# ArrowLuo/SegCLIP

Measured on AMD Instinct MI355X. Metric: image-text pairs/s fwd+bwd, ViT-B/16 224^2, per-GPU batch 256 (global 2048 at 8 GPUs), higher is better.
Workload: dtype bf16; 1 GPU; BASELINE configs[1]/[2]: ViT-B/16 224^2 + 77-token text, contrastive loss only; per_gpu_batch=256, global_batch=256, parallelism=dp1, attention_forward=bf16, residual_stream=fp32, cross_mode=t18, text_positions=all 77 (full context, as the reference computes it)

## Files before the change

### include/segclip_hip.h

```cpp
#ifndef SEGCLIP_HIP_H
#define SEGCLIP_HIP_H

#include <stddef.h>
#include <stdint.h>

#ifdef __cplusplus
extern "C" {
#endif

#define SEGCLIP_ABI_VERSION 1

#define SEGCLIP_F32 0
#define SEGCLIP_BF16 1

#define SEGCLIP_ACT_NONE 0
#define SEGCLIP_ACT_QUICK_GELU 1
#define SEGCLIP_ACT_GELU_ERF 2

#define SEGCLIP_ERR_INVALID (-1)
#define SEGCLIP_ERR_UNSUPPORTED (-2)

int segclip_version(void);
const char* segclip_last_error_string(void);

// ... 68 lines not shown
int segclip_layernorm_fwd_multi(const void* x, int n, const float* const* gamma, const float* const* beta,
                                void* const* y, const int64_t* maps, float* mean, float* rstd, int64_t rows,
                                int64_t cols, float eps, int x_dtype, int y_dtype, void* stream);
size_t segclip_layernorm_bwd_multi_ws_bytes(int64_t rows, int64_t cols, int n);
int segclip_layernorm_bwd_multi(const void* const* dy, const void* x, int n, const float* const* gamma,
                                const int64_t* maps, const float* mean, const float* rstd, void* dx, float* dgb,
                                void* ws, int64_t rows, int64_t cols, int dy_dtype, int x_dtype, void* stream);

#define SEGCLIP_ATTN_FP8 1
typedef struct segclip_attn_desc {
  const void* Q;
  const void* K;
  const void* V;
  void* O;
  void* stats;
  const void* dO;
  void* dQ;
  void* dK;
  void* dV;
  void* ws;
  int64_t B, H, Tq, Tk, hd;
  int64_t q_sb, q_st, k_sb, k_st, v_sb, v_st, o_sb, o_st;
  int64_t dq_sb, dq_st, dk_sb, dk_st, dv_sb, dv_st, do_sb, do_st;
  float scale;
  int32_t causal;
  int32_t dtype;
  int32_t flags;
  void* colsum_part;
  const int32_t* klen;
} segclip_attn_desc;

size_t segclip_attn_stats_bytes(const segclip_attn_desc* d);
size_t segclip_attn_bwd_ws_bytes(const segclip_attn_desc* d);
int segclip_attn_fwd(const segclip_attn_desc* d, void* stream);
int segclip_attn_bwd(const segclip_attn_desc* d, void* stream);

typedef struct segclip_resblock_fwd_desc {
  const void* x;
  const float* ln1w; const float* ln1b; const void* wqkv; const float* bqkv; const void* wo; const float* bo;
  const float* ln2w; const float* ln2b; const void* wfc; const float* bfc; const void* wpr; const float* bpr;
  void* y1; float* mean1; float* rstd1;
  void* qkv;
  void* o;
  void* stats;
  void* x1;
  void* y2; float* mean2; float* rstd2;
  void* h; int64_t ld_h;
  void* u; int64_t ld_u;
  void* xo;
  const void* klen;
  int64_t M, B, T, D, F, H;
  float eps, attn_scale;
  int32_t causal, act, aux_kind, x_dtype;
} segclip_resblock_fwd_desc;
int segclip_resblock_fwd(const segclip_resblock_fwd_desc* d, void* stream);

int segclip_cast(const void* src, void* dst, int64_t n, int src_dtype, int dst_dtype, void* stream);
int segclip_split3_bf16(const float* src, void* dst, int64_t rows, int64_t cols, int64_t ld, int stack, int role, void* stream);
size_t segclip_colsum_ws_bytes(int64_t M, int64_t N);
int segclip_colsum(const void* X, float* out, void* ws, int64_t M, int64_t N, int64_t ld, int dtype,
                   void* stream);
int segclip_act_fwd(const void* x, void* y, int64_t n, int act, int dtype, void* stream);
int segclip_act_bwd(const void* dy, const void* x, void* dx, int64_t n, int act, int dtype, void* stream);
int segclip_add(const void* a, const void* b, void* out, int64_t n, int dtype, void* stream);

int segclip_im2col(const float* image, void* cols, int64_t B, int64_t C, int64_t H, int64_t W, int64_t p,
                   int layout, int out_dtype, void* stream);
int segclip_im2col_ld(const float* image, void* cols, int64_t B, int64_t C, int64_t H, int64_t W, int64_t p,
                      int layout, int out_dtype, int64_t ld, void* stream);
int segclip_vis_assemble(const void* patches, const float* cls, const float* pos, float* x, int64_t B,
                         int64_t T, int64_t D, int p_dtype, void* stream);

int segclip_embed_fwd(const int64_t* ids, const float* table, const float* pos, float* out, int64_t B,
                      int64_t L, int64_t D, int64_t vocab, void* stream);
int segclip_embed_bwd(const int64_t* ids, const float* dout, float* dtable, float* dpos, int64_t B,
                      int64_t L, int64_t D, int64_t vocab, void* stream);

int segclip_mean_cat_fwd(const float* x, float* out, int64_t B, int64_t T, int64_t D, void* stream);
int segclip_mean_cat_bwd(const float* dout, float* dx, int64_t B, int64_t T, int64_t D, void* stream);
int segclip_mae_unshuffle_fwd(const float* x, const float* mask_token, const int64_t* ids, const float* pos, float* out, int64_t B,
                              int64_t K, int64_t L, int64_t D, void* stream);
int segclip_mae_unshuffle_bwd(const float* dout, const int64_t* ids, float* dx, float* dpos, float* mpart, int64_t B, int64_t K,
                              int64_t L, int64_t D, void* stream);

int segclip_gather_rows(const void* src, const int64_t* idx, void* out, int64_t B, int64_t Tsrc,
                        int64_t Tout, int64_t D, int dtype, void* stream);
int segclip_scatter_rows(const void* dout, const int64_t* idx, void* dsrc, int64_t B, int64_t Tsrc,
                         int64_t Tout, int64_t D, int dtype, void* stream);

int segclip_assign_fwd(const float* logits, const float* gumbel, float tau, float* y_soft, float* soft,
                       uint8_t* idx, float* hard, float* counts, int64_t B, int64_t G, int64_t T,
                       void* stream);
int segclip_assign_bwd(const float* dhard, const float* y_soft, float tau, float* dlogits, int64_t B,
                       int64_t G, int64_t T, void* stream);

int segclip_l2norm_fwd(const float* x, float* y, float* norm, int64_t rows, int64_t cols, void* stream);
int segclip_l2norm_bwd(const float* dy, const float* y, const float* norm, float* dx, int64_t rows,
                       int64_t cols, void* stream);
int segclip_ce_fwd(const float* logits, float* lse, float* loss_rows, int64_t rows, int64_t cols,
                   int64_t label_offset, void* stream);
int segclip_ce_bwd(const float* logits, const float* lse, const float* gscale_ptr, float gscale,
                   float* dlogits, int64_t rows, int64_t cols, int64_t label_offset, void* stream);
int segclip_ce_labels_fwd(const float* logits, const int64_t* labels, int64_t ignore_index, float* lse, float* loss_rows,
                          float* valid, int64_t rows, int64_t cols, void* stream);
int segclip_ce_labels_bwd(const float* logits, const float* lse, const int64_t* labels, int64_t ignore_index,
                          const float* gscale, const float* inv_count, float* dlogits, int64_t rows, int64_t cols,
                          void* stream);
int segclip_superpixel_kl(const float* hard, const int64_t* seg, float* loss_rows, float* dhard,
// ... 330 lines not shown
```

### segclip_amd/config.py

```python
import contextlib
import sys
import threading
import types

import torch

_warned_env = set()


def tuning_env(name, default):
    import os
    v = os.environ.get(name)
    if v is None:
        return default
    if os.environ.get("SEGCLIP_TUNING", "0") in ("", "0"):
        if name not in _warned_env:
            _warned_env.add(name)
            print(f"segclip_amd: {name}={v} ignored (tuning switches need SEGCLIP_TUNING=1)", file=sys.stderr)
        return default
    return v


_DEFAULTS = dict(compute_dtype=torch.float32, f32_split=False, c_exec=tuning_env("SEGCLIP_C_EXEC", "1") != "0", cross_mode="t18", overlap_towers=True,
                 trust_weight_shadows=False, attn_fp8=False, fuse_res_stack=True, bf16_resgrad=True, bf16_resid=False, fused_head=True,
                 aux_u8=tuning_env("SEGCLIP_AUX_U8", "1") != "0",
                 text_after_blocks=3, text_trim=False, text_trim_hint=None, pad_rows=tuning_env("SEGCLIP_PAD_ROWS", "1") != "0", fold_param_grads=tuning_env("SEGCLIP_FOLD_GRADS", "1") != "0",
                 wgrad_group_blocks=int(tuning_env("SEGCLIP_WGRAD_GROUP", "12")), wgrad_group_blocks_dist=int(tuning_env("SEGCLIP_WGRAD_GROUP_DIST", "12")))
_tls = threading.local()


def _get(name):
    ov = getattr(_tls, "overrides", None)
    if ov:
        for d in reversed(ov):
            if name in d:
                return d[name]
    return _DEFAULTS[name]


def _check(name, value):
    if name == "compute_dtype" and value not in (torch.float32, torch.bfloat16):
        raise ValueError("compute dtype must be torch.float32 or torch.bfloat16")
    if name == "cross_mode" and value not in ("t18", "intended"):
        raise ValueError("cross_mode must be 't18' or 'intended'")
    return value


class _ConfigModule(types.ModuleType):
    """Module type whose switches are properties: reads resolve thread-local overrides first, writes set the
    process default."""


for _n in _DEFAULTS:
    setattr(_ConfigModule, _n, property(lambda self, _n=_n: _get(_n),
                                        lambda self, v, _n=_n: _DEFAULTS.__setitem__(_n, _check(_n, v))))
sys.modules[__name__].__class__ = _ConfigModule


def set_compute_dtype(dtype):
    _DEFAULTS["compute_dtype"] = _check("compute_dtype", dtype)


def set_cross_mode(mode):
    _DEFAULTS["cross_mode"] = _check("cross_mode", mode)


@contextlib.contextmanager
def scope(**overrides):
    for k, v in overrides.items():
        if k not in _DEFAULTS:
            raise KeyError(f"unknown switch {k!r}")
        _check(k, v)
    stack = getattr(_tls, "overrides", None)
    if stack is None:
        stack = _tls.overrides = []
    stack.append(dict(overrides))
    try:
        yield
    finally:
        stack.pop()


def set_stack_hook(after_blocks, fn):
    _tls.stack_hook = (int(after_blocks), fn)


def take_stack_hook():
    h = getattr(_tls, "stack_hook", None)
    _tls.stack_hook = None
    return h


@contextlib.contextmanager
def noise_injection(items):
    prev = getattr(_tls, "noise", None)
    _tls.noise = list(items)
    try:
        yield
    finally:
        _tls.noise = prev


def _take(kind, shape, device):
    noise = getattr(_tls, "noise", None)
    if noise is None:
        return None
    if not noise:
        raise RuntimeError("noise_injection: more noise draws than injected tensors")
    k, t = noise.pop(0)
    if k != kind or tuple(t.shape) != tuple(shape):
        raise RuntimeError(f"noise_injection: expected {kind}{tuple(shape)}, got {k}{tuple(t.shape)}")
    return t.to(device=device, dtype=torch.float32)


def gumbel(shape, device):
    t = _take("gumbel", shape, device)
    if t is not None:
        return t
    u = torch.rand(shape, device=device, dtype=torch.float32)
    if u.is_cuda:
        from . import _lib as L
        L.check(L.load().segclip_gumbel_from_uniform(L.ptr(u), L.ptr(u), u.numel(), L.stream()), "gumbel_from_uniform")
        return u
    tiny = torch.finfo(torch.float32).tiny
    u = u.clamp(min=tiny, max=1.0 - torch.finfo(torch.float32).eps)
    return -torch.log(-torch.log(u))


def rand(shape, device):
    t = _take("rand", shape, device)
    if t is not None:
        return t
    return torch.rand(shape, device=device, dtype=torch.float32)
```

### segclip_amd/csrc/exec.cpp

```cpp
#include <initializer_list>

#include "common.h"
#include "gemm_plan.h"

namespace {

void gemm_base(segclip_gemm_desc& g, const void* A, int64_t lda, const void* W, int64_t ldw, void* Cc, int64_t ldc, int c_dtype,
               const float* bias, int64_t M, int64_t N, int64_t K) {
  g = segclip_gemm_desc{};
  g.A = A; g.B = W; g.C = Cc; g.bias = bias;
  g.M = M; g.N = N; g.K = K;
  g.sam = lda; g.sak = 1; g.sbn = ldw; g.sbk = 1;
  g.ldc = ldc; g.ldaux = N;
  g.nb1 = 1; g.nb2 = 1;
  g.a_dtype = SEGCLIP_BF16; g.b_dtype = SEGCLIP_BF16; g.c_dtype = c_dtype; g.r_dtype = SEGCLIP_F32;
  g.act = SEGCLIP_ACT_NONE; g.alpha = 1.0f;
}

}

extern "C" int segclip_resblock_fwd(const segclip_resblock_fwd_desc* d, void* stream) {
  SEGCLIP_REQUIRE(d != nullptr, "resblock_fwd: null descriptor");
  SEGCLIP_REQUIRE(d->M >= d->B * d->T && d->B > 0 && d->T > 0 && d->D > 0 && d->F > 0 && d->H > 0 && d->D % d->H == 0,
                  "resblock_fwd: bad sizes");
  SEGCLIP_REQUIRE(d->x && d->y1 && d->qkv && d->o && d->stats && d->x1 && d->y2 && d->h && d->xo && d->mean1 && d->rstd1 &&
                  d->mean2 && d->rstd2, "resblock_fwd: null buffer");
  SEGCLIP_REQUIRE(d->x_dtype == SEGCLIP_F32 || d->x_dtype == SEGCLIP_BF16, "resblock_fwd: residual stream must be f32 or bf16");
  const int64_t M = d->M, D = d->D, F = d->F, hd = D / d->H;
  segclip_gemm_desc in_proj, out_proj, c_fc, c_proj;
  gemm_base(in_proj, d->y1, D, d->wqkv, D, d->qkv, 3 * D, SEGCLIP_BF16, d->bqkv, M, 3 * D, D);
  gemm_base(out_proj, d->o, D, d->wo, D, d->x1, D, d->x_dtype, d->bo, M, D, D);
  out_proj.residual = d->x; out_proj.ldr = D; out_proj.r_dtype = d->x_dtype;
  gemm_base(c_fc, d->y2, D, d->wfc, D, d->h, d->ld_h, SEGCLIP_BF16, d->bfc, M, F, D);
  c_fc.act = d->act; c_fc.aux = d->u; c_fc.ldaux = d->u ? d->ld_u : F; c_fc.aux_kind = d->aux_kind;
  gemm_base(c_proj, d->h, d->ld_h, d->wpr, F, d->xo, D, d->x_dtype, d->bpr, M, D, F);
  c_proj.residual = d->x1; c_proj.ldr = D; c_proj.r_dtype = d->x_dtype;
  int rc;
  for (const segclip_gemm_desc* g : {&in_proj, &out_proj, &c_fc, &c_proj})
    if ((rc = gemm_plan(g).rc)) return rc;
  rc = segclip_layernorm_fwd(d->x, d->ln1w, d->ln1b, d->y1, d->mean1, d->rstd1, M, D, d->eps, d->x_dtype, SEGCLIP_BF16, stream);
  if (rc) return rc;
  if ((rc = segclip_gemm(&in_proj, stream))) return rc;
  if (M > d->B * d->T) {
    hipError_t e = hipMemsetAsync((char*)d->o + (size_t)d->B * d->T * D * 2, 0, (size_t)(M - d->B * d->T) * D * 2, (hipStream_t)stream);
    SEGCLIP_REQUIRE(e == hipSuccess, "resblock_fwd: memset failed: %s", hipGetErrorString(e));
  }
  segclip_attn_desc a = segclip_attn_desc{};
  a.Q = d->qkv; a.K = (const char*)d->qkv + (size_t)D * 2; a.V = (const char*)d->qkv + (size_t)2 * D * 2; a.O = d->o;
  a.stats = d->stats;
  a.B = d->B; a.H = d->H; a.Tq = d->T; a.Tk = d->T; a.hd = hd;
  a.q_sb = a.k_sb = a.v_sb = d->T * 3 * D; a.q_st = a.k_st = a.v_st = 3 * D;
  a.o_sb = d->T * D; a.o_st = D;
  a.scale = d->attn_scale; a.causal = d->causal; a.dtype = SEGCLIP_BF16; a.flags = 0;
  a.klen = (decltype(a.klen))d->klen;
  if ((rc = segclip_attn_fwd(&a, stream))) return rc;
  if ((rc = segclip_gemm(&out_proj, stream))) return rc;
  rc = segclip_layernorm_fwd(d->x1, d->ln2w, d->ln2b, d->y2, d->mean2, d->rstd2, M, D, d->eps, d->x_dtype, SEGCLIP_BF16, stream);
  if (rc) return rc;
  if ((rc = segclip_gemm(&c_fc, stream))) return rc;
  return segclip_gemm(&c_proj, stream);
}
```

### segclip_amd/modules/modeling.py

```python
from functools import partial

import torch
from torch import nn

from .. import _lib as L
from .. import config, ops
from .module_clip import CLIP, available_models
from .module_mae import MAEDecoder
from .util_module import CrossEn, PreTrainedModel, dist_collect, get_attr, get_logger, show_log


def _detached(obj):
    if isinstance(obj, torch.Tensor):
        return obj.detach()
    if isinstance(obj, dict):
        return {k: _detached(v) for k, v in obj.items()}
    if isinstance(obj, (list, tuple)):
        return type(obj)(_detached(v) for v in obj)
    return obj


class SegCLIPPreTrainedModel(PreTrainedModel, nn.Module):
    def __init__(self, *inputs, **kwargs):
        super().__init__()
# ... 75 lines not shown
        mae_vis_mask_ratio = get_attr(task_config, "mae_vis_mask_ratio", default_value=0.75)
        self.use_vision_mae_recon = get_attr(task_config, "use_vision_mae_recon", default_value=False)
        if self.use_vision_mae_recon:
            self.vis_mask_ratio = mae_vis_mask_ratio
            self.vis_mae_decoder = MAEDecoder(vision_width, vision_width // 2, image_resolution, vision_patch_size,
                                              decoder_depth=3, decoder_num_heads=8, mlp_ratio=4.,
                                              norm_layer=partial(nn.LayerNorm, eps=1e-6))
        mae_seq_mask_ratio = get_attr(task_config, "mae_seq_mask_ratio", default_value=0.15)
        self.use_text_mae_recon = get_attr(task_config, "use_text_mae_recon", default_value=False)
        if self.use_text_mae_recon:
            self.seq_mask_ratio = mae_seq_mask_ratio
            self.seq_mae_decoder = MAEDecoder(embed_dim, embed_dim // 2, image_resolution, vision_patch_size,
                                              decoder_depth=3, decoder_num_heads=8, mlp_ratio=4., choice_seq=True,
                                              pred_len=vocab_size, seq_len=self.task_config.max_words)
        self.use_seglabel = get_attr(task_config, "use_seglabel", default_value=False)
        self.apply(self.init_weights)
        self.segclip_config = {}

    def scope(self):
        return config.scope(**self.segclip_config)

    def _text_stream(self):
        from .. import streams
        return streams.side_stream("text")

    def _visual_feature(self, image, image_frame):
        if config.fused_head:
            return self.clip.encode_image_pooled(image)
        visual_output, _hidden, mid_states = self.get_visual_output(image, shaped=True, image_frame=image_frame, return_hidden=True)
        return visual_output, mid_states

    def forward(self, input_ids, token_type_ids, attention_mask, image, image_seg=None):
        if self.segclip_config:
            with config.scope(**self.segclip_config):
                return self._forward(input_ids, token_type_ids, attention_mask, image, image_seg)
        return self._forward(input_ids, token_type_ids, attention_mask, image, image_seg)

    def _forward(self, input_ids, token_type_ids, attention_mask, image, image_seg=None):
        input_ids = input_ids.view(-1, input_ids.shape[-1])
        L.require_cuda(input_ids, torch.as_tensor(image))
        image_input = torch.as_tensor(image).float()
        b, pair, channel, h, w = image_input.shape
        image = image_input[:, 0].reshape(b, channel, h, w)
        image_frame = 1
        if not self.training:
            return None
        ops._GradFold.advance()
        if config.compute_dtype == torch.bfloat16:
            ops.refresh_weight_shadows(force=not config.trust_weight_shadows)
        if config.overlap_towers:
            main = torch.cuda.current_stream()
            side = self._text_stream()
            ready = torch.cuda.Event()
            ready.record(main)
            box = {}

            def enqueue_text():
                side.wait_event(ready)
                with torch.cuda.stream(side):
                    box["seq"] = self.clip.encode_text_eot(input_ids).unsqueeze(1)
            k = int(config.text_after_blocks)
            if k > 0:
                config.set_stack_hook(k, enqueue_text)
            else:
                enqueue_text()
            pending = None
            try:
                visual_output, mid_states = self._visual_feature(image, image_frame)
                pending = config.take_stack_hook()
            finally:
                config.take_stack_hook()
            if pending is not None:
                pending[1]()
            sequence_output = box["seq"]
            main.wait_stream(side)
            sequence_output.record_stream(main)
        else:
            sequence_output = self.clip.encode_text_eot(input_ids).unsqueeze(1)
            visual_output, mid_states = self._visual_feature(image, image_frame)
        self.last_mid_states = _detached(mid_states)
        self._last_head = {}
        if config.fused_head:
            loss = ops.ClipLossFn.apply(visual_output.float().view(b, -1), sequence_output.squeeze(1).float(),
                                        self.clip.logit_scale, int(getattr(self.task_config, "rank", 0)), self._last_head)
        else:
            sim_matrix_t2v, sim_matrix_v2t = self._loose_similarity(sequence_output, visual_output)
            offset = sequence_output.size(0) * int(getattr(self.task_config, "rank", 0))
            sim_loss1 = ops.CrossEntropyFn.apply(sim_matrix_t2v, offset)
            sim_loss2 = ops.CrossEntropyFn.apply(sim_matrix_v2t, offset)
            loss = (sim_loss1 + sim_loss2) / 2.
            self._last_head["logits"] = (sim_matrix_t2v.detach(), sim_matrix_v2t.detach())
        self.last_losses = {"contrastive": loss.detach()}
        if self.use_seglabel:
            image_seg_ = torch.as_tensor(image_seg)[:, 0].reshape(b, -1)
            hard = mid_states["attns"][0]["hard_attn"]
            clutering_loss = ops.SuperpixelKLFn.apply(hard, image_seg_)
            loss = loss + clutering_loss
            self.last_losses["kl"] = clutering_loss.detach()
        if self.use_text_mae_recon:
            attention_mask = attention_mask.view(-1, attention_mask.shape[-1])
            _, seq_hidden, seq_mae_mask, seq_mae_ids_restore = self.get_sequence_output(
                input_ids, token_type_ids, attention_mask, shaped=True, return_hidden=True, mask_ratio=self.seq_mask_ratio)
            seq_mae_mask = seq_mae_mask.view(-1, seq_mae_mask.size(-1))
            seq_mae_ids_restore = seq_mae_ids_restore.view(-1, seq_mae_ids_restore.size(-1))
            _mae_mask = (seq_mae_mask + attention_mask).gt(1)
            self.last_text_mae = _detached((seq_mae_mask, seq_mae_ids_restore, seq_hidden))
            seq_mae_loss = self.seq_mae_decoder.forward_seq(input_ids, seq_hidden, _mae_mask, seq_mae_ids_restore,
                                                            attention_mask)
            loss = loss + seq_mae_loss
            self.last_losses["text_mae"] = seq_mae_loss.detach()
        if self.use_vision_mae_recon:
            _, vis_hidden, vis_mae_mask, vis_mae_ids_restore, mid_mae_states = self.get_visual_output(
                image, shaped=True, image_frame=image_frame, return_hidden=True, mask_ratio=self.vis_mask_ratio)
            vis_hidden = mid_mae_states["hidden"]
            vis_hidden = ops.mean_cat(vis_hidden)
            vis_mae_mask = vis_mae_mask.view(-1, vis_mae_mask.size(-1))
            vis_mae_ids_restore = vis_mae_ids_restore.view(-1, vis_mae_ids_restore.size(-1))
            self.last_mae = _detached((vis_mae_mask, vis_mae_ids_restore, mid_mae_states))
            vis_mae_loss = self.vis_mae_decoder.forward_vis(image, vis_hidden, vis_mae_mask, vis_mae_ids_restore,
                                                            loss_allpatch=False)
            loss = loss + vis_mae_loss
            self.last_losses["mae"] = vis_mae_loss.detach()
        return loss

    @property
# ... 85 lines not shown
```

### segclip_amd/ops.py

```python
import collections
import ctypes as C
import math
import os
import weakref

import torch
import torch.distributed as dist
from torch.autograd import Function

from . import _lib as L
from . import config as _cfg

ACT_NONE, ACT_QUICK_GELU, ACT_GELU_ERF = L.ACT_NONE, L.ACT_QUICK_GELU, L.ACT_GELU_ERF


class _GemmProfile:
    enabled = False
    records = []

    @classmethod
    def start(cls):
        cls.enabled, cls.records = True, []

    @classmethod
# ... 874 lines not shown
    try:
        L.check(L.load().segclip_resblock_fwd(C.byref(d), L.stream()), "resblock_fwd")
    except L.Unsupported:
        return False
    return True


def _resblock_fwd(x2, P, B, T, n_head, causal, act, eps, act_dtype, klen):
    P = BlockParams._make(P)
    M, D = x2.shape
    F4 = P.wfc.shape[0]
    for w in P:
        sl = _slot_of(w)
        if sl is not None:
            sl.note_forward_use()
    bf = act_dtype == torch.bfloat16
    fp8 = bf and bool(_cfg.attn_fp8)
    wqkv_c, wo_c, wfc_c, wpr_c = (wcast(w, act_dtype) for w in (P.wqkv, P.wo, P.wfc, P.wpr))
    ak = _aux_kind(act_dtype, act, M, F4)
    hidden = _empty_pitched if bf else _empty
    y1, y2, o = (_empty((M, D), act_dtype, x2) for _ in range(3))
    qkv = _empty((M, 3 * D), act_dtype, x2)
    mean1, rstd1, mean2, rstd2 = _empty((4, M), torch.float32, x2).unbind(0)
    x1, xo = _empty((M, D), x2.dtype, x2), _empty((M, D), x2.dtype, x2)
    h = hidden((M, F4), act_dtype, x2)
    u = hidden((M, F4), torch.uint8 if ak == 2 else act_dtype, x2) if act != ACT_NONE else None
    ad = attn_desc_packed(qkv, o, B, n_head, T, causal, klen=klen, fp8=fp8)
    stats = _empty((max(L.load().segclip_attn_stats_bytes(C.byref(ad)) // 4, 1),), torch.float32, x2)
    s = BlockSaved(x=x2, ln1w=P.ln1w, mean1=mean1, rstd1=rstd1, y1=y1, wqkv=wqkv_c, qkv=qkv, o=o, stats=stats, wo=wo_c, x1=x1,
                   ln2w=P.ln2w, mean2=mean2, rstd2=rstd2, y2=y2, wfc=wfc_c, u=u, h=h, wpr=wpr_c)
    if (bf and _cfg.c_exec and not _OpCount.enabled and not _GemmProfile.enabled and not fp8 and x2.is_contiguous() and D % 8 == 0
            and _resblock_fwd_exec(s, P, xo, B, T, n_head, causal, act, eps, klen, ak)):
        return xo, s
    p_ln_fwd(x2, P.ln1w, P.ln1b, eps, act_dtype, out=y1, stats=(mean1, rstd1))
    p_linear(y1, wqkv_c, P.bqkv, out=qkv)
    if M > B * T:
        o[B * T:].zero_()
    p_attn_fwd(ad, x2, stats=stats)
    p_linear(o, wo_c, P.bo, residual=x2, out=x1)
    p_ln_fwd(x1, P.ln2w, P.ln2b, eps, act_dtype, out=y2, stats=(mean2, rstd2))
    _, u = p_linear(y2, wfc_c, P.bfc, act=act, want_aux=True, aux_kind=ak, pitched=bf, out=h, aux_out=u)
    p_linear(h, wpr_c, P.bpr, residual=x1, out=xo)
    return xo, s._replace(u=u)


def _aux_kind(act_dtype, act, M=0, N=0):
    if act_dtype == torch.bfloat16 and act in (ACT_QUICK_GELU, ACT_GELU_ERF):
        if _cfg.aux_u8 and M > 0 and M % 128 == 0 and N % 256 == 0:
            return 2
        return 1 if act == ACT_QUICK_GELU else 0
    return 0


def _resblock_bwd(s, cfg, klen, slots, need, g, g16, chain, wgroup=None, rqueue=None):
    B, T, D, n_head, causal, act, act_dtype = cfg
    M = s.x.shape[0]
    bf = act_dtype == torch.bfloat16
    if bf and g16 is None:
        g16 = p_cast(g, act_dtype)
    if not bf:
        g16 = g
    res_in = g16 if chain else g
    rdt = act_dtype if chain else torch.float32
    F4 = s.wfc.shape[0]

    rq = ReduceQueue() if rqueue is None else rqueue

    def wgrad(dy_, x_, out_):
        if wgroup is not None:
            return wgroup.add(dy_, x_, out_)
        return p_wgrad(dy_, x_, out=out_, defer=rq)

    def vec_out(slot, wanted, n):
        return _slot_out(slot, (n,)) if wanted else None
    du, dbfc = p_dgrad(g16, s.wpr, act_dtype, aux=s.u, act=act, want_colsum=True, colsum_out=vec_out(slots.bfc, need.bfc, F4),
                       aux_kind=2 if s.u.dtype == torch.uint8 else _aux_kind(act_dtype, act),
                       defer=rq, pitched=bf)
    dwpr = wgrad(g16, s.h, _slot_out(slots.wpr, (D, F4))) if need.wpr else None
    dy2 = p_dgrad(du, s.wfc, act_dtype)
    dwfc = wgrad(du, s.y2, _slot_out(slots.wfc, (F4, D))) if need.wfc else None
    two = bf and not chain
    r = p_ln_bwd(dy2, s.x1, s.ln2w, s.mean2, s.rstd2, dres=res_in, dx_dtype=rdt, want_bf16=two, want_dres_colsum=True,
                 outs=(vec_out(slots.ln2w, need.ln2w, D), vec_out(slots.ln2b, need.ln2b, D), vec_out(slots.bpr, need.bpr, D)), defer=rq)
    dx1, dln2w, dln2b = r[0], r[1], r[2]
    dx1_16 = r[3] if two else dx1
    dbpr = r[-1] if need.bpr else None
    do = p_dgrad(dx1_16, s.wo, act_dtype)
    dwo = wgrad(dx1_16, s.o, _slot_out(slots.wo, (D, D))) if need.wo else None
    dqkv = _empty((M, 3 * D), act_dtype, s.x)
    if M > B * T:
        dqkv[B * T:].zero_()
    s3 = (T * 3 * D, 3 * D)
    ad = attn_desc_packed(s.qkv, s.o, B, n_head, T, causal, klen=klen)
    part = _empty((B, 3 * D), torch.float32, s.x) if (bf and need.bqkv) else None
    p_attn_bwd(ad, s.stats, do, dqkv, dqkv, dqkv, s3, s3, s3, (T * D, D), 0, D, 2 * D, colsum_part=part)
    dy1 = p_dgrad(dqkv, s.wqkv, act_dtype)
    dwqkv = wgrad(dqkv, s.y1, _slot_out(slots.wqkv, (3 * D, D))) if need.wqkv else None
    dbqkv = None
    if need.bqkv:
        bq_out = _slot_out(slots.bqkv, (3 * D,))
        if part is not None and (bq_out is None or bq_out.data_ptr() % 16 == 0):
            dbqkv = bq_out if bq_out is not None else _empty((3 * D,), torch.float32, s.x)
            rq.add_rows(part, B, 3 * D, 3 * D, (dbqkv,), 3 * D)
        else:
            dbqkv = p_colsum(part if part is not None else dqkv, out=bq_out)
    r = p_ln_bwd(dy1, s.x, s.ln1w, s.mean1, s.rstd1, dres=dx1, dx_dtype=rdt, want_bf16=two, want_dres_colsum=True,
                 outs=(vec_out(slots.ln1w, need.ln1w, D), vec_out(slots.ln1b, need.ln1b, D), vec_out(slots.bo, need.bo, D)), defer=rq)
    if rqueue is None:
        rq.flush()
    dbo = r[-1] if need.bo else None
    dx32 = None if chain else r[0]
    dx16 = r[0] if chain else (r[3] if two else None)
    return dx32, dx16, BlockParams(ln1w=r[1], ln1b=r[2], wqkv=dwqkv, bqkv=dbqkv, wo=dwo, bo=dbo, ln2w=dln2w, ln2b=dln2b, wfc=dwfc,
                                   bfc=dbfc, wpr=dwpr, bpr=dbpr)


def _bf16_side_copy(g):
    st = getattr(g, "_segclip_bf16", None)
    if st is not None and (st.numel() != g.numel() or st.device != g.device or not g.is_contiguous()):
        return None
    return st


def _pad_rows(t, Mp):
    M = t.shape[0]
    padded = _empty((Mp, t.shape[1]), t.dtype, t)
    padded[:M].copy_(t)
    padded[M:].zero_()
    return padded


class ResBlockFn(Function):

    @staticmethod
    def forward(ctx, x, ln1w, ln1b, wqkv, bqkv, wo, bo, ln2w, ln2b, wfc, bfc, wpr, bpr, n_head, causal, act, eps,
                act_dtype, klen=None):
        B, T, D = x.shape
        x2 = x.contiguous().view(B * T, D)
        P = BlockParams(ln1w, ln1b, wqkv, bqkv, wo, bo, ln2w, ln2b, wfc, bfc, wpr, bpr)
        xo, saved = _resblock_fwd(x2, P, B, T, n_head, causal, act, eps, act_dtype, klen)
        ctx.save_for_backward(*saved)
        ctx.cfg = (B, T, D, n_head, causal, act, act_dtype)
        ctx.klen = klen
        ctx.slots = BlockParams._make(_slot_of(w) for w in P)
        _GradFold.other[id(ln1w)] = weakref.ref(ln1w)
        return xo.view(B, T, D)

    @staticmethod
    def backward(ctx, g):
        B, T, D, n_head, causal, act, act_dtype = ctx.cfg
        M = B * T
        st = _bf16_side_copy(g)
        g = g.contiguous().view(M, D)
        g16 = st.view(M, D) if (st is not None and act_dtype == torch.bfloat16) else None
        (need,) = _block_records(BlockParams, ctx.needs_input_grad, start=1, count=1)
        dx, dx16, grads = _resblock_bwd(BlockSaved._make(ctx.saved_tensors), ctx.cfg, ctx.klen, ctx.slots, need, g, g16, False)
        dx = dx.view(B, T, D)
        if dx16 is not None:
            dx._segclip_bf16 = dx16.view(B, T, D)
        return (dx,) + grads + (None, None, None, None, None, None)


class _GradFold:
    epoch = 0
    armed = -1
    first = {}
    uses = {}
    other = {}

    @classmethod
    def advance(cls):
        cls.epoch += 1
        cls.first.clear()
        cls.uses.clear()
        cls.other.clear()

    @classmethod
    def used_elsewhere(cls, p):
        r = cls.other.get(id(p))
        return r is not None and r() is p

    @classmethod
    def take(cls, p, gr, adds):
        if gr is None or gr.dtype != torch.float32 or not gr.is_contiguous():
            return gr
        ent = cls.first.get(id(p))
        if ent is not None and ent[0] == cls.epoch and ent[1].shape == gr.shape and ent[1].device == gr.device:
            adds.append((ent[1], gr))
            return None
        cls.first[id(p)] = (cls.epoch, gr.detach())
        if cls.armed != cls.epoch:
            cls.armed = cls.epoch
            torch.autograd.Variable._execution_engine.queue_callback(cls.advance)
        return gr

    @staticmethod
    def flush(adds):
        if not adds:
            return
        n = len(adds)
        dst = (C.c_void_p * n)(*[d.data_ptr() for d, _ in adds])
        src = (C.c_void_p * n)(*[s_.data_ptr() for _, s_ in adds])
        cnt = (C.c_int64 * n)(*[d.numel() for d, _ in adds])
        L.check(L.load().segclip_multi_add_f32(C.cast(dst, C.c_void_p), C.cast(src, C.c_void_p), C.cast(cnt, C.c_void_p), n,
                                               L.stream()), "multi_add_f32")
        adds.clear()


class ResStackFn(Function):

    NP = len(BlockParams._fields)

    @staticmethod
    def forward(ctx, x, n_head, causal, act, eps, act_dtype, klen, chain, keep16, *params):
        B, T, D = x.shape
        blocks = _block_records(BlockParams, params)
        cur = x.contiguous().view(B * T, D)
        M = B * T
        Mp = 128 * -(-M // 128) if (act_dtype == torch.bfloat16 and bool(_cfg.pad_rows) and M % 128 != 0 and M >= _PAD_ROWS_MIN) else M
        ctx.Mp = Mp
        ctx.in_dtype = x.dtype
        resid16 = act_dtype == torch.bfloat16 and (bool(_cfg.bf16_resid) or x.dtype == torch.bfloat16)
        if resid16 and cur.dtype != torch.bfloat16:
            cur = p_cast(cur, torch.bfloat16)
        elif not resid16 and cur.dtype != torch.float32:
            cur = p_cast(cur, torch.float32)
        if Mp != M:
            cur = _pad_rows(cur, Mp)
        saved = []
        for P in blocks:
            cur, sv = _resblock_fwd(cur, P, B, T, n_head, causal, act, eps, act_dtype, klen)
            saved.extend(sv)
        if Mp != M:
            cur = cur[:M]
        ctx.save_for_backward(*saved)
        ctx.cfg = (B, T, D, n_head, causal, act, act_dtype)
        ctx.klen = klen
        ctx.chain = (bool(chain) or resid16) and act_dtype == torch.bfloat16
        ctx.wgrad_group, ctx.wgrad_group_dist = int(_cfg.wgrad_group_blocks), int(_cfg.wgrad_group_blocks_dist)
        ctx.fold = bool(_cfg.fold_param_grads) and len(params) > 0
        if ctx.fold:
            for P in blocks:
                k = id(P.ln1w)
                _GradFold.uses[k] = _GradFold.uses.get(k, 0) + 1
        ctx.blocks = blocks
        ctx.slots = [BlockParams._make(_slot_of(w) for w in P) for P in blocks]
        if resid16 and not keep16:
            cur = p_cast(cur, torch.float32)
        return cur.view(B, T, D)

    @staticmethod
    def backward(ctx, g):
        B, T, D, n_head, causal, act, act_dtype = ctx.cfg
        M, nblk = B * T, len(ctx.blocks)
        Mp = ctx.Mp
        bf = act_dtype == torch.bfloat16
        st = _bf16_side_copy(g)
        g = g.contiguous().view(M, D)
        if Mp != M:
            st = None
            g, M = _pad_rows(g, Mp), Mp
        cur16 = st.view(M, D) if (st is not None and bf) else None
        if bf and cur16 is None and g.dtype == torch.bfloat16:
            cur16 = g
        if ctx.chain and cur16 is None:
            cur16 = p_cast(g, act_dtype)
        cur32 = None if ctx.chain else (g if g.dtype == torch.float32 else p_cast(g, torch.float32))
        saved = _block_records(BlockSaved, ctx.saved_tensors)
        needs = _block_records(BlockParams, ctx.needs_input_grad, start=len(ctx.needs_input_grad) - nblk * ResStackFn.NP)
        out = [None] * nblk
        wg, sizes = None, []
        if ctx.wgrad_group > 1 and ctx.cfg[-1] == torch.bfloat16 and nblk > 1:
            Dm, F4 = ctx.blocks[0].wqkv.shape[1], ctx.blocks[0].wfc.shape[0]
            if Dm % 256 == 0 and F4 % 256 == 0 and Mp % 64 == 0:
                no_slots = all(s is None for sl in ctx.slots for s in sl)
                gmax = ctx.wgrad_group if no_slots else min(ctx.wgrad_group, ctx.wgrad_group_dist)
                tiles_blk = (4 * Dm * Dm + 2 * F4 * Dm) // 65536
                sizes = wgrad_group_plan(nblk, tiles_blk, Mp // 64, gmax)
                wg = WgradGroup() if max(sizes) > 1 else None
        left = sizes.pop(0) if wg is not None else 0
        grq = ReduceQueue() if wg is not None else None
        pending = []
        adds = []
        for b in reversed(range(nblk)):
            cur32, cur16, grads = _resblock_bwd(saved[b], ctx.cfg, ctx.klen, ctx.slots[b], needs[b], cur32, cur16, ctx.chain, wg, grq)
            pending.append((b, ctx.blocks[b], ctx.slots[b], grads))
            if wg is not None:
                left -= 1
                if left > 0 and b > 0:
                    continue
                wg.flush()
                if grq is not None:
                    grq.flush()
                left = sizes.pop(0) if sizes else nblk
            for b_, P_, sl_, grads_ in pending:
                fold = ctx.fold and _GradFold.uses.get(id(P_.ln1w), 0) > 1 and not _GradFold.used_elsewhere(P_.ln1w)
                given = out[b_] = list(grads_)
                for i, (p, gr, slot) in enumerate(zip(P_, grads_, sl_)):
                    if gr is None:
                        continue
                    owner = slot.owner() if slot is not None else None
                    if owner is not None and gr.data_ptr() == slot.ptr and p.grad is None and slot.single_use():
                        p.grad = gr
                        owner._on_grad(p)
                        given[i] = None
                    elif fold and slot is None:
                        given[i] = _GradFold.take(p, gr, adds)
            pending = []
        _GradFold.flush(adds)
        if Mp != B * T:
            cur16 = cur16[:B * T] if cur16 is not None else None
            cur32 = cur32[:B * T] if cur32 is not None else None
        if ctx.chain and ctx.in_dtype == torch.bfloat16:
            dx = cur16
        elif ctx.chain:
            dx = p_cast(cur16, torch.float32)
        else:
            dx = cur32
        dx = dx.view(B, T, D)
        if cur16 is not None and dx.dtype != torch.bfloat16:
            dx._segclip_bf16 = cur16.view(B, T, D)
        return (dx, None, None, None, None, None, None, None, None) + tuple(gr for given in out for gr in given)


def res_stack(x, blocks_params, n_head, causal, act, eps, act_dtype, klen=None, keep16=False):
    flat = [p for P in blocks_params for p in P]
    keep16 = bool(keep16) and bool(_cfg.bf16_resid) and act_dtype == torch.bfloat16
    return ResStackFn.apply(x, n_head, causal, act, eps, act_dtype, klen, bool(_cfg.bf16_resgrad), keep16, *flat)


def _cross_attn_desc(qp, kv, o, B, G, S, n_head, mode):
    D = qp.shape[1]
    hd = D // n_head
    qs = (G * D, D)
    ks = (2 * D, B * 2 * D) if mode == "t18" else (S * 2 * D, 2 * D)
    return _attn_desc(qp, kv, kv, o, B, n_head, G, S, hd, qs, ks, ks, qs, 1.0 / math.sqrt(hd), False, 0, 0, D), qs, ks


# ... 1762 lines not shown
```

Measured before the change: 7273 pairs/s.

## Add C-side residual block backward executor and gate text tower launch on block count

Adds a C entry point that runs the whole residual-block backward (dgrad GEMMs, layernorm backward, attention backward) from one descriptor, so the Python path issues one call per block instead of many. Weight-gradient GEMMs and column reductions stay in Python. Separately, the side-stream text encoder is now enqueued only after the visual forward, and its ready event is recorded after a set number of visual blocks (default 7) instead of at the start. This moves the tower overlap point and adds a new descriptor ABI plus per-call buffer allocations.

```diff
diff --git a/include/segclip_hip.h b/include/segclip_hip.h
--- a/include/segclip_hip.h
+++ b/include/segclip_hip.h
@@ -144,8 +144,26 @@
   int64_t M, B, T, D, F, H;
   float eps, attn_scale;
   int32_t causal, act, aux_kind, x_dtype;
+  const void* g16;
+  const void* gres;
+  void* du; int64_t ld_du;
+  float* dbfc; float* dbfc_part;
+  void* dy2;
+  void* dx1; void* dx1_16;
+  float* ln2_part;
+  void* dattn;
+  void* dqkv;
+  float* bqkv_part;
+  void* dy1;
+  void* dx; void* dx_16;
+  float* ln1_part;
+  void* ws; int64_t ws_bytes;
+  int32_t g_dtype, reserved;
 } segclip_resblock_fwd_desc;
 int segclip_resblock_fwd(const segclip_resblock_fwd_desc* d, void* stream);
+
+size_t segclip_resblock_bwd_ws_bytes(const segclip_resblock_fwd_desc* d);
+int segclip_resblock_bwd(const segclip_resblock_fwd_desc* d, void* stream);
 
 int segclip_cast(const void* src, void* dst, int64_t n, int src_dtype, int dst_dtype, void* stream);
 int segclip_split3_bf16(const float* src, void* dst, int64_t rows, int64_t cols, int64_t ld, int stack, int role, void* stream);
diff --git a/segclip_amd/config.py b/segclip_amd/config.py
--- a/segclip_amd/config.py
+++ b/segclip_amd/config.py
@@ -24,7 +24,7 @@
 _DEFAULTS = dict(compute_dtype=torch.float32, f32_split=False, c_exec=tuning_env("SEGCLIP_C_EXEC", "1") != "0", cross_mode="t18", overlap_towers=True,
                  trust_weight_shadows=False, attn_fp8=False, fuse_res_stack=True, bf16_resgrad=True, bf16_resid=False, fused_head=True,
                  aux_u8=tuning_env("SEGCLIP_AUX_U8", "1") != "0",
-                 text_after_blocks=3, text_trim=False, text_trim_hint=None, pad_rows=tuning_env("SEGCLIP_PAD_ROWS", "1") != "0", fold_param_grads=tuning_env("SEGCLIP_FOLD_GRADS", "1") != "0",
+                 text_after_blocks=3, text_gate_blocks=int(tuning_env("SEGCLIP_TEXT_GATE", "7")), text_trim=False, text_trim_hint=None, pad_rows=tuning_env("SEGCLIP_PAD_ROWS", "1") != "0", fold_param_grads=tuning_env("SEGCLIP_FOLD_GRADS", "1") != "0",
                  wgrad_group_blocks=int(tuning_env("SEGCLIP_WGRAD_GROUP", "12")), wgrad_group_blocks_dist=int(tuning_env("SEGCLIP_WGRAD_GROUP_DIST", "12")))
 _tls = threading.local()
 
@@ -91,6 +91,25 @@
     return h
 
 
+def set_block_mark(after_blocks, fn):
+    _tls.block_mark = [int(after_blocks), fn]
+
+
+def block_tick():
+    m = getattr(_tls, "block_mark", None)
+    if m is not None:
+        m[0] -= 1
+        if m[0] <= 0:
+            _tls.block_mark = None
+            m[1]()
+
+
+def take_block_mark():
+    m = getattr(_tls, "block_mark", None)
+    _tls.block_mark = None
+    return m
+
+
 @contextlib.contextmanager
 def noise_injection(items):
     prev = getattr(_tls, "noise", None)
diff --git a/segclip_amd/csrc/exec.cpp b/segclip_amd/csrc/exec.cpp
--- a/segclip_amd/csrc/exec.cpp
+++ b/segclip_amd/csrc/exec.cpp
@@ -60,3 +60,103 @@
   if ((rc = segclip_gemm(&c_fc, stream))) return rc;
   return segclip_gemm(&c_proj, stream);
 }
+
+namespace {
+
+constexpr size_t WS_ALIGN = 256;
+size_t ws_round(size_t n) { return (n + WS_ALIGN - 1) / WS_ALIGN * WS_ALIGN; }
+
+struct BlockBwd {
+  segclip_gemm_desc c_proj, c_fc, out_proj, in_proj;
+  segclip_attn_desc attn;
+  size_t off_fc, off_o, off_qkv, off_attn, ws_bytes;
+};
+
+void dgrad_base(segclip_gemm_desc& g, const void* dy, int64_t ld_dy, const void* w, void* dx, int64_t ld_dx, int64_t M, int64_t N,
+                int64_t K) {
+  gemm_base(g, dy, ld_dy, w, 1, dx, ld_dx, SEGCLIP_BF16, nullptr, M, N, K);
+  g.sbk = N;
+}
+
+void describe_bwd(BlockBwd& k, const segclip_resblock_fwd_desc* d) {
+  const int64_t M = d->M, D = d->D, F = d->F;
+  dgrad_base(k.c_proj, d->g16, D, d->wpr, d->du, d->ld_du, M, F, D);
+  k.c_proj.aux = d->u; k.c_proj.ldaux = d->ld_u; k.c_proj.act = d->act; k.c_proj.mul_dact = 1; k.c_proj.aux_kind = d->aux_kind;
+  k.c_proj.colsum = d->dbfc; k.c_proj.colsum_ws = d->dbfc_part; k.c_proj.flags = SEGCLIP_GEMM_DEFER_COLSUM;
+  dgrad_base(k.c_fc, d->du, d->ld_du, d->wfc, d->dy2, D, M, D, F);
+  dgrad_base(k.out_proj, d->dx1_16 ? d->dx1_16 : d->dx1, D, d->wo, d->dattn, D, M, D, D);
+  dgrad_base(k.in_proj, d->dqkv, 3 * D, d->wqkv, d->dy1, D, M, D, 3 * D);
+  segclip_attn_desc& a = k.attn;
+  a = segclip_attn_desc{};
+  a.Q = d->qkv; a.K = (const char*)d->qkv + (size_t)D * 2; a.V = (const char*)d->qkv + (size_t)2 * D * 2; a.O = d->o;
+  a.stats = d->stats; a.colsum_part = d->bqkv_part;
+  a.dO = d->dattn; a.dQ = d->dqkv; a.dK = (char*)d->dqkv + (size_t)D * 2; a.dV = (char*)d->dqkv + (size_t)2 * D * 2;
+  a.B = d->B; a.H = d->H; a.Tq = d->T; a.Tk = d->T; a.hd = D / d->H;
+  a.q_sb = a.k_sb = a.v_sb = a.dq_sb = a.dk_sb = a.dv_sb = d->T * 3 * D;
+  a.q_st = a.k_st = a.v_st = a.dq_st = a.dk_st = a.dv_st = 3 * D;
+  a.o_sb = a.do_sb = d->T * D; a.o_st = a.do_st = D;
+  a.scale = d->attn_scale; a.causal = d->causal; a.dtype = SEGCLIP_BF16; a.flags = 0;
+  a.klen = (decltype(a.klen))d->klen;
+  size_t off = 0;
+  size_t* const offs[3] = {&k.off_fc, &k.off_o, &k.off_qkv};
+  segclip_gemm_desc* const plain[3] = {&k.c_fc, &k.out_proj, &k.in_proj};
+  for (int i = 0; i < 3; ++i) {
+    const size_t n = gemm_splitk_ws_bytes(plain[i]);
+    *offs[i] = off;
+    if (n && d->ws) { plain[i]->ws = (char*)d->ws + off; plain[i]->ws_bytes = (int64_t)n; }
+    off += ws_round(n);
+  }
+  k.off_attn = off;
+  const size_t n = segclip_attn_bwd_ws_bytes(&a);
+  if (d->ws) a.ws = (char*)d->ws + off;
+  k.ws_bytes = off + ws_round(n > 4 ? n : 4);
+}
+
+bool bwd_sizes_ok(const segclip_resblock_fwd_desc* d) {
+  return d->M >= d->B * d->T && d->B > 0 && d->T > 0 && d->D > 0 && d->F > 0 && d->H > 0 && d->D % d->H == 0;
+}
+
+}
+
+extern "C" size_t segclip_resblock_bwd_ws_bytes(const segclip_resblock_fwd_desc* d) {
+  if (d == nullptr || !bwd_sizes_ok(d)) return 0;
+  BlockBwd k;
+  describe_bwd(k, d);
+  return k.ws_bytes;
+}
+
+extern "C" int segclip_resblock_bwd(const segclip_resblock_fwd_desc* d, void* stream) {
+  SEGCLIP_REQUIRE(d != nullptr, "resblock_bwd: null descriptor");
+  SEGCLIP_REQUIRE(bwd_sizes_ok(d), "resblock_bwd: bad sizes");
+  SEGCLIP_REQUIRE(d->x && d->ln1w && d->mean1 && d->rstd1 && d->wqkv && d->qkv && d->o && d->stats && d->wo && d->x1 && d->ln2w &&
+                  d->mean2 && d->rstd2 && d->wfc && d->u && d->wpr, "resblock_bwd: null saved buffer");
+  SEGCLIP_REQUIRE(d->g16 && d->gres && d->du && d->dbfc && d->dbfc_part && d->dy2 && d->dx1 && d->ln2_part && d->dattn && d->dqkv &&
+                  d->dy1 && d->dx && d->ln1_part && d->ws, "resblock_bwd: null gradient buffer");
+  SEGCLIP_REQUIRE(d->x_dtype == SEGCLIP_F32 || d->x_dtype == SEGCLIP_BF16, "resblock_bwd: residual stream must be f32 or bf16");
+  SEGCLIP_REQUIRE(d->g_dtype == SEGCLIP_F32 || d->g_dtype == SEGCLIP_BF16, "resblock_bwd: residual gradient must be f32 or bf16");
+  SEGCLIP_REQUIRE(d->g_dtype == SEGCLIP_BF16 ? (d->gres == d->g16 && !d->dx1_16 && !d->dx_16) : (d->dx1_16 != nullptr),
+                  "resblock_bwd: bf16 residual gradients are their own GEMM operands, fp32 ones need dx1_16");
+  BlockBwd k;
+  describe_bwd(k, d);
+  SEGCLIP_REQUIRE((size_t)d->ws_bytes >= k.ws_bytes, "resblock_bwd: workspace of %lld bytes, %lld needed", (long long)d->ws_bytes,
+                  (long long)k.ws_bytes);
+  const int64_t M = d->M, D = d->D;
+  int rc;
+  for (const segclip_gemm_desc* g : {&k.c_proj, &k.c_fc, &k.out_proj, &k.in_proj})
+    if ((rc = gemm_plan(g).rc)) return rc;
+  if ((rc = segclip_gemm(&k.c_proj, stream))) return rc;
+  if ((rc = segclip_gemm(&k.c_fc, stream))) return rc;
+  rc = segclip_layernorm_bwd(d->dy2, d->x1, d->ln2w, d->mean2, d->rstd2, d->gres, d->dx1, d->dx1_16, nullptr, nullptr, nullptr,
+                             d->ln2_part, M, D, SEGCLIP_BF16, d->x_dtype, d->g_dtype, stream);
+  if (rc) return rc;
+  if ((rc = segclip_gemm(&k.out_proj, stream))) return rc;
+  if (M > d->B * d->T) {
+    hipError_t e = hipMemsetAsync((char*)d->dqkv + (size_t)d->B * d->T * 3 * D * 2, 0, (size_t)(M - d->B * d->T) * 3 * D * 2,
+                                  (hipStream_t)stream);
+    SEGCLIP_REQUIRE(e == hipSuccess, "resblock_bwd: memset failed: %s", hipGetErrorString(e));
+  }
+  if ((rc = segclip_attn_bwd(&k.attn, stream))) return rc;
+  if ((rc = segclip_gemm(&k.in_proj, stream))) return rc;
+  return segclip_layernorm_bwd(d->dy1, d->x, d->ln1w, d->mean1, d->rstd1, d->dx1, d->dx, d->dx_16, nullptr, nullptr, nullptr,
+                               d->ln1_part, M, D, SEGCLIP_BF16, d->x_dtype, d->g_dtype, stream);
+}
diff --git a/segclip_amd/modules/modeling.py b/segclip_amd/modules/modeling.py
--- a/segclip_amd/modules/modeling.py
+++ b/segclip_amd/modules/modeling.py
@@ -151,7 +151,9 @@
             main = torch.cuda.current_stream()
             side = self._text_stream()
             ready = torch.cuda.Event()
-            ready.record(main)
+            gate = int(config.text_gate_blocks)
+            if gate <= 0:
+                ready.record(main)
             box = {}
 
             def enqueue_text():
@@ -159,17 +161,27 @@
                 with torch.cuda.stream(side):
                     box["seq"] = self.clip.encode_text_eot(input_ids).unsqueeze(1)
             k = int(config.text_after_blocks)
-            if k > 0:
+            if gate > 0:
+                config.set_block_mark(gate, lambda: ready.record(main))
+                if k > 0:
+                    config.set_stack_hook(k, lambda: None)
+            elif k > 0:
                 config.set_stack_hook(k, enqueue_text)
             else:
                 enqueue_text()
-            pending = None
+            pending = mark = None
             try:
                 visual_output, mid_states = self._visual_feature(image, image_frame)
                 pending = config.take_stack_hook()
+                mark = config.take_block_mark()
             finally:
                 config.take_stack_hook()
-            if pending is not None:
+                config.take_block_mark()
+            if gate > 0:
+                if mark is not None:
+                    mark[1]()
+                enqueue_text()
+            elif pending is not None:
                 pending[1]()
             sequence_output = box["seq"]
             main.wait_stream(side)
diff --git a/segclip_amd/ops.py b/segclip_amd/ops.py
--- a/segclip_amd/ops.py
+++ b/segclip_amd/ops.py
@@ -950,7 +950,60 @@
     return 0
 
 
-def _resblock_bwd(s, cfg, klen, slots, need, g, g16, chain, wgroup=None, rqueue=None):
+BlockBwdBufs = collections.namedtuple("BlockBwdBufs", "du dbfc dbfc_part dy2 dx1 dx1_16 ln2_part dattn dqkv part dy1 dx dx_16 ln1_part "
+                                                      "ln_rows ws")
+
+
+def _resblock_bwd_exec(s, cfg, klen, g16, res_in, rdt, two, want_part, ak, dbfc_out):
+    B, T, D, n_head, causal, act, act_dtype = cfg
+    M, F4 = s.x.shape[0], s.wfc.shape[0]
+    if not all(t.is_contiguous() for t in (s.x, s.x1, s.qkv, s.o, s.wqkv, s.wo, s.wfc, s.wpr)) or s.u.stride(1) != 1:
+        return None
+    lib = L.load()
+    L.require_cuda(s.x, g16, res_in)
+    lnb = lib.segclip_layernorm_bwd_ws_bytes(M, D)
+    u8 = lambda n: torch.empty(max(n, 4), dtype=torch.uint8, device=s.x.device)
+    md = lambda dtype: _empty((M, D), dtype, s.x)
+    b = BlockBwdBufs(
+        du=_empty_pitched((M, F4), act_dtype, s.x), dbfc=dbfc_out if dbfc_out is not None else _empty((F4,), torch.float32, s.x),
+        dbfc_part=_empty((max(M // 64, 1), F4), torch.float32, s.x), dy2=md(act_dtype), dx1=md(rdt),
+        dx1_16=md(torch.bfloat16) if two else None, ln2_part=u8(lnb), dattn=md(act_dtype), dqkv=_empty((M, 3 * D), act_dtype, s.x),
+        part=_empty((B, 3 * D), torch.float32, s.x) if want_part else None, dy1=md(act_dtype), dx=md(rdt),
+        dx_16=md(torch.bfloat16) if two else None, ln1_part=u8(lnb), ln_rows=lnb // (3 * D * 4), ws=None)
+    d = L.ResBlockFwdDesc()
+    d.x, d.x1, d.qkv, d.o, d.stats = s.x.data_ptr(), s.x1.data_ptr(), s.qkv.data_ptr(), s.o.data_ptr(), s.stats.data_ptr()
+    d.ln1w, d.mean1, d.rstd1 = s.ln1w.data_ptr(), s.mean1.data_ptr(), s.rstd1.data_ptr()
+    d.ln2w, d.mean2, d.rstd2 = s.ln2w.data_ptr(), s.mean2.data_ptr(), s.rstd2.data_ptr()
+    d.wqkv, d.wo, d.wfc, d.wpr = s.wqkv.data_ptr(), s.wo.data_ptr(), s.wfc.data_ptr(), s.wpr.data_ptr()
+    d.u, d.ld_u = s.u.data_ptr(), s.u.stride(0)
+    if klen is not None:
+        if klen.dtype != torch.int32 or klen.numel() != B or not klen.is_contiguous():
+            raise TypeError("attention: klen must be a contiguous int32 tensor of B entries")
+        L.require_cuda(klen)
+        d.klen = klen.data_ptr()
+    d.M, d.B, d.T, d.D, d.F, d.H = M, B, T, D, F4, n_head
+    d.attn_scale = 1.0 / math.sqrt(D // n_head)
+    d.causal, d.act, d.aux_kind, d.x_dtype = int(causal), int(act), int(ak), L.dt(s.x)
+    d.g16, d.gres, d.g_dtype = g16.data_ptr(), res_in.data_ptr(), L.dt(res_in)
+    d.du, d.ld_du, d.dbfc, d.dbfc_part = b.du.data_ptr(), b.du.stride(0), b.dbfc.data_ptr(), b.dbfc_part.data_ptr()
+    d.dy2, d.dx1, d.ln2_part = b.dy2.data_ptr(), b.dx1.data_ptr(), b.ln2_part.data_ptr()
+    d.dattn, d.dqkv, d.dy1 = b.dattn.data_ptr(), b.dqkv.data_ptr(), b.dy1.data_ptr()
+    d.dx, d.ln1_part = b.dx.data_ptr(), b.ln1_part.data_ptr()
+    if two:
+        d.dx1_16, d.dx_16 = b.dx1_16.data_ptr(), b.dx_16.data_ptr()
+    if b.part is not None:
+        d.bqkv_part = b.part.data_ptr()
+    d.ws_bytes = lib.segclip_resblock_bwd_ws_bytes(C.byref(d))
+    b = b._replace(ws=u8(d.ws_bytes))
+    d.ws = b.ws.data_ptr()
+    try:
+        L.check(lib.segclip_resblock_bwd(C.byref(d), L.stream()), "resblock_bwd")
+    except L.Unsupported:
+        return None
+    return b
+
+
+def _resblock_bwd(s, cfg, klen, slots, need, g, g16, chain, wgroup=None, rqueue=None, c_exec=False):
     B, T, D, n_head, causal, act, act_dtype = cfg
     M = s.x.shape[0]
     bf = act_dtype == torch.bfloat16
@@ -971,15 +1024,48 @@
 
     def vec_out(slot, wanted, n):
         return _slot_out(slot, (n,)) if wanted else None
-    du, dbfc = p_dgrad(g16, s.wpr, act_dtype, aux=s.u, act=act, want_colsum=True, colsum_out=vec_out(slots.bfc, need.bfc, F4),
-                       aux_kind=2 if s.u.dtype == torch.uint8 else _aux_kind(act_dtype, act),
+    two = bf and not chain
+    ak = 2 if s.u.dtype == torch.uint8 else _aux_kind(act_dtype, act)
+    dbfc_out = vec_out(slots.bfc, need.bfc, F4)
+    ln2_outs = (vec_out(slots.ln2w, need.ln2w, D), vec_out(slots.ln2b, need.ln2b, D), vec_out(slots.bpr, need.bpr, D))
+    ln1_outs = (vec_out(slots.ln1w, need.ln1w, D), vec_out(slots.ln1b, need.ln1b, D), vec_out(slots.bo, need.bo, D))
+    want_part = bf and need.bqkv
+    if (bf and c_exec and not _OpCount.enabled and not _GemmProfile.enabled and M > 0 and fused_colsum_ok(M, F4, D, act_dtype)
+            and g16.is_contiguous() and res_in.is_contiguous() and res_in.dtype == rdt
+            and all(t is None or t.data_ptr() % 16 == 0 for t in ln2_outs + ln1_outs)):
+        e = _resblock_bwd_exec(s, cfg, klen, g16, res_in, rdt, two, want_part, ak, dbfc_out)
+        if e is not None:
+            vec = lambda out: out if out is not None else _empty((D,), torch.float32, s.x)
+            rq.add_rows(e.dbfc_part, M // 64, F4, F4, (e.dbfc,), F4)
+            dwpr = wgrad(g16, s.h, _slot_out(slots.wpr, (D, F4))) if need.wpr else None
+            dwfc = wgrad(e.du, s.y2, _slot_out(slots.wfc, (F4, D))) if need.wfc else None
+            dln2w, dln2b, dbpr = (vec(o) for o in ln2_outs)
+            rq.add_rows(e.ln2_part, e.ln_rows, 3 * D, 3 * D, (dln2w, dln2b, dbpr), D)
+            dx1_16 = e.dx1_16 if two else e.dx1
+            dwo = wgrad(dx1_16, s.o, _slot_out(slots.wo, (D, D))) if need.wo else None
+            dwqkv = wgrad(e.dqkv, s.y1, _slot_out(slots.wqkv, (3 * D, D))) if need.wqkv else None
+            dbqkv = None
+            if need.bqkv:
+                bq_out = _slot_out(slots.bqkv, (3 * D,))
+                if bq_out is None or bq_out.data_ptr() % 16 == 0:
+                    dbqkv = bq_out if bq_out is not None else _empty((3 * D,), torch.float32, s.x)
+                    rq.add_rows(e.part, B, 3 * D, 3 * D, (dbqkv,), 3 * D)
+                else:
+                    dbqkv = p_colsum(e.part, out=bq_out)
+            dln1w, dln1b, dbo = (vec(o) for o in ln1_outs)
+            rq.add_rows(e.ln1_part, e.ln_rows, 3 * D, 3 * D, (dln1w, dln1b, dbo), D)
+            if rqueue is None:
+                rq.flush()
+            return (None if chain else e.dx, e.dx if chain else e.dx_16,
+                    BlockParams(ln1w=dln1w, ln1b=dln1b, wqkv=dwqkv, bqkv=dbqkv, wo=dwo, bo=dbo if need.bo else None, ln2w=dln2w,
+                                ln2b=dln2b, wfc=dwfc, bfc=e.dbfc, wpr=dwpr, bpr=dbpr if need.bpr else None))
+    du, dbfc = p_dgrad(g16, s.wpr, act_dtype, aux=s.u, act=act, want_colsum=True, colsum_out=dbfc_out, aux_kind=ak,
                        defer=rq, pitched=bf)
     dwpr = wgrad(g16, s.h, _slot_out(slots.wpr, (D, F4))) if need.wpr else None
     dy2 = p_dgrad(du, s.wfc, act_dtype)
     dwfc = wgrad(du, s.y2, _slot_out(slots.wfc, (F4, D))) if need.wfc else None
-    two = bf and not chain
     r = p_ln_bwd(dy2, s.x1, s.ln2w, s.mean2, s.rstd2, dres=res_in, dx_dtype=rdt, want_bf16=two, want_dres_colsum=True,
-                 outs=(vec_out(slots.ln2w, need.ln2w, D), vec_out(slots.ln2b, need.ln2b, D), vec_out(slots.bpr, need.bpr, D)), defer=rq)
+                 outs=ln2_outs, defer=rq)
     dx1, dln2w, dln2b = r[0], r[1], r[2]
     dx1_16 = r[3] if two else dx1
     dbpr = r[-1] if need.bpr else None
@@ -990,7 +1076,7 @@
         dqkv[B * T:].zero_()
     s3 = (T * 3 * D, 3 * D)
     ad = attn_desc_packed(s.qkv, s.o, B, n_head, T, causal, klen=klen)
-    part = _empty((B, 3 * D), torch.float32, s.x) if (bf and need.bqkv) else None
+    part = _empty((B, 3 * D), torch.float32, s.x) if want_part else None
     p_attn_bwd(ad, s.stats, do, dqkv, dqkv, dqkv, s3, s3, s3, (T * D, D), 0, D, 2 * D, colsum_part=part)
     dy1 = p_dgrad(dqkv, s.wqkv, act_dtype)
     dwqkv = wgrad(dqkv, s.y1, _slot_out(slots.wqkv, (3 * D, D))) if need.wqkv else None
@@ -1003,7 +1089,7 @@
         else:
             dbqkv = p_colsum(part if part is not None else dqkv, out=bq_out)
     r = p_ln_bwd(dy1, s.x, s.ln1w, s.mean1, s.rstd1, dres=dx1, dx_dtype=rdt, want_bf16=two, want_dres_colsum=True,
-                 outs=(vec_out(slots.ln1w, need.ln1w, D), vec_out(slots.ln1b, need.ln1b, D), vec_out(slots.bo, need.bo, D)), defer=rq)
+                 outs=ln1_outs, defer=rq)
     if rqueue is None:
         rq.flush()
     dbo = r[-1] if need.bo else None
@@ -1037,9 +1123,11 @@
         x2 = x.contiguous().view(B * T, D)
         P = BlockParams(ln1w, ln1b, wqkv, bqkv, wo, bo, ln2w, ln2b, wfc, bfc, wpr, bpr)
         xo, saved = _resblock_fwd(x2, P, B, T, n_head, causal, act, eps, act_dtype, klen)
+        _cfg.block_tick()
         ctx.save_for_backward(*saved)
         ctx.cfg = (B, T, D, n_head, causal, act, act_dtype)
         ctx.klen = klen
+        ctx.c_exec = bool(_cfg.c_exec)
         ctx.slots = BlockParams._make(_slot_of(w) for w in P)
         _GradFold.other[id(ln1w)] = weakref.ref(ln1w)
         return xo.view(B, T, D)
@@ -1052,7 +1140,7 @@
         g = g.contiguous().view(M, D)
         g16 = st.view(M, D) if (st is not None and act_dtype == torch.bfloat16) else None
         (need,) = _block_records(BlockParams, ctx.needs_input_grad, start=1, count=1)
-        dx, dx16, grads = _resblock_bwd(BlockSaved._make(ctx.saved_tensors), ctx.cfg, ctx.klen, ctx.slots, need, g, g16, False)
+        dx, dx16, grads = _resblock_bwd(BlockSaved._make(ctx.saved_tensors), ctx.cfg, ctx.klen, ctx.slots, need, g, g16, False, c_exec=ctx.c_exec)
         dx = dx.view(B, T, D)
         if dx16 is not None:
             dx._segclip_bf16 = dx16.view(B, T, D)
@@ -1129,6 +1217,7 @@
         for P in blocks:
             cur, sv = _resblock_fwd(cur, P, B, T, n_head, causal, act, eps, act_dtype, klen)
             saved.extend(sv)
+            _cfg.block_tick()
         if Mp != M:
             cur = cur[:M]
         ctx.save_for_backward(*saved)
@@ -1136,6 +1225,7 @@
         ctx.klen = klen
         ctx.chain = (bool(chain) or resid16) and act_dtype == torch.bfloat16
         ctx.wgrad_group, ctx.wgrad_group_dist = int(_cfg.wgrad_group_blocks), int(_cfg.wgrad_group_blocks_dist)
+        ctx.c_exec = bool(_cfg.c_exec)
         ctx.fold = bool(_cfg.fold_param_grads) and len(params) > 0
         if ctx.fold:
             for P in blocks:
@@ -1181,7 +1271,7 @@
         pending = []
         adds = []
         for b in reversed(range(nblk)):
-            cur32, cur16, grads = _resblock_bwd(saved[b], ctx.cfg, ctx.klen, ctx.slots[b], needs[b], cur32, cur16, ctx.chain, wg, grq)
+            cur32, cur16, grads = _resblock_bwd(saved[b], ctx.cfg, ctx.klen, ctx.slots[b], needs[b], cur32, cur16, ctx.chain, wg, grq, ctx.c_exec)
             pending.append((b, ctx.blocks[b], ctx.slots[b], grads))
             if wg is not None:
                 left -= 1
```

New measurement: 7334 pairs/s (median of 6 runs). About the same (+0.8%).
